# roahmlab/koopman-realizations

Measured on AMD Instinct MI355X. Metric: EDMD snapshot-pairs/sec (bilinear fit, 3-link arm, poly-3), higher is better.
Workload: dtype f64

## Files before the change

### koopman-realizations_amd/_ffi.py

```python
from __future__ import annotations

import ctypes as C
import os

import numpy as np

_HERE = os.path.dirname(os.path.abspath(__file__))
LIB_PATH = os.environ.get("KP_LIB_PATH") or os.path.join(_HERE, "libkoopman_hip.so")

KP_OK, KP_ERR_ARG, KP_ERR_HIP, KP_ERR_NOT_SPD, KP_ERR_QP_FAIL, KP_ERR_NOT_CONVERGED = 0, -1, -2, -3, -4, -5
MODEL = {"linear": 0, "bilinear": 1, "nonlinear": 2}
BLOCK = {"poly": 0, "fourier": 1, "gaussian": 2, "hermite": 3, "fourier_sparser": 4}
LIFT_FULL, LIFT_ECON, LIFT_ROW = 0, 1, 2

c_dp = C.POINTER(C.c_double)
c_ip = C.POINTER(C.c_int)
vp = C.c_void_p


class KpBasisDesc(C.Structure):
    _fields_ = [("model_type", C.c_int32), ("nzeta", C.c_int32), ("m", C.c_int32), ("n_blocks", C.c_int32),
                ("block_type", C.POINTER(C.c_int32)), ("block_count", C.POINTER(C.c_int32)),
                ("poly_exps", C.POINTER(C.c_uint8)), ("gauss_centres", c_dp),
                ("k_pcs", C.c_int32), ("pcs", c_dp)]
# ... 104 lines not shown
    "kp_nmpc_destroy": (C.c_int, [vp]),
}
TIMER_NMPC_SIM = 21

OBSERVER_SIGNATURES = {
    "kp_load_observe": (C.c_int, [vp, vp, C.c_int, c_dp, c_dp, C.c_int, C.c_int64, c_dp, c_dp, C.c_int,
                                  C.POINTER(C.c_int64), C.c_int64, C.POINTER(C.c_int32), C.POINTER(C.c_int64), C.c_int, c_dp,
                                  C.c_int, c_dp, c_dp, c_ip]),
}
OBS_RATE, OBS_PIN_LAST = 1, 2

CT_SIGNATURES = {
    "kp_logm": (C.c_int, [vp, C.c_int, C.c_int, c_dp, C.c_double, C.c_double, c_dp, c_ip, c_ip]),
    "kp_rollout_ct": (C.c_int, [vp, C.c_int, C.c_int, c_dp, c_dp, C.c_int, C.c_int, c_dp, c_dp, C.c_int, C.c_int, C.c_double,
                                C.c_double, C.c_double, c_dp, c_ip, c_ip, c_ip]),
    "kp_rollout_nl_ct": (C.c_int, [vp, vp, C.c_int, c_dp, c_dp, c_dp, C.c_int, C.c_double, C.c_double, C.c_double, c_dp, c_ip, c_ip,
                                   c_ip]),
}

class KpArmParams(C.Structure):
    _fields_ = [("Nmods", C.c_int), ("nlinks", C.c_int), ("l", C.c_double), ("k", C.c_double), ("d", C.c_double),
                ("m", C.c_double), ("i", C.c_double), ("g", C.c_double), ("ku", C.c_double)]


ARM_SIGNATURES = {
    "kp_arm_simulate": (C.c_int, [vp, C.POINTER(KpArmParams), C.c_int, C.c_int, C.c_int, c_dp, C.c_double, c_dp, c_dp, c_dp,
                                  C.c_double, C.c_double, c_dp, c_ip, c_ip, c_ip]),
}
ARM_MODE = {"zoh": 0, "interp": 1, "floor": 2, "restart": 3}

class KpRsysDims(C.Structure):
    _fields_ = [("num_terms", C.c_int), ("degree_x", C.c_int), ("degree_u", C.c_int)]


RSYS_SIGNATURES = {
    "kp_rsys_simulate": (C.c_int, [vp, C.POINTER(KpRsysDims), C.c_int, C.c_int, C.c_int, C.c_int, c_dp, c_dp, c_ip, c_ip, c_dp,
                                   c_dp, c_dp, C.c_int, C.c_double, C.c_double, c_dp, c_ip, c_ip, c_ip, C.POINTER(vp)]),
}
RSYS_MODE = {"span": 0, "restart": 1}

VALIDATE_SIGNATURES = {
    "kp_validate": (C.c_int, [vp, vp, C.c_int, C.c_int, C.c_int, C.c_int, C.c_int, C.c_int, C.c_int, c_dp, c_dp, C.c_int,
                              C.POINTER(C.c_int64), c_dp, c_dp, c_dp, c_dp, c_dp, C.c_int, c_dp, c_ip, c_dp]),
    "kp_validate_ct": (C.c_int, [vp, vp, C.c_int, C.c_int, C.c_int, C.c_int, C.c_int, C.c_int, C.c_int, c_dp, c_dp, C.c_int,
                                 C.POINTER(C.c_int64), c_dp, c_dp, c_dp, c_dp, c_dp, C.c_int, C.c_double, C.c_double, C.c_double,
                                 c_dp, c_ip, c_dp, c_ip, c_ip]),
}
HORIZON_SIGNATURES = {
    "kp_validate_horizon": (C.c_int, [vp, vp, C.c_int, C.c_int, C.c_int, C.c_int, C.c_int, C.c_int, c_dp, c_dp, C.c_int,
                                      C.POINTER(C.c_int64), c_dp, c_dp, c_dp, C.c_int, C.c_int, c_dp, C.POINTER(C.c_int64), c_ip]),
}
TIMER_HORIZON = 24
TIMER_HORIZON_TILE = 25
HORIZON_CHUNK = 8
VALIDATE_CHUNK = 128
VALIDATE_CT_CHUNK = 32
VALIDATE_CT_STAGE = 8192

SIM_SIGNATURES = {
    "kp_mpc_simulate": (C.c_int, [vp, vp, C.c_int, C.c_int, c_dp, C.c_int, c_dp, c_dp, C.c_int, c_dp, c_dp, c_dp, c_ip, c_ip]),
}
TIMER_MPC_SIM = 19

SPECTRUM_SIGNATURES = {
    "kp_eig": (C.c_int, [vp, C.c_int, C.c_int, c_dp, C.c_int, c_dp, c_dp, c_dp, c_ip, c_ip]),
}
TIMER_EIG = 22
TIMER_EIG_REGIME = 23
EIG_MAXN = 512
EIG_WAVE_MAX = 32
EIG_LDS_MAXN_VEC, EIG_LDS_MAXN_VAL = 99, 140

_lib = None


def lib():
    global _lib
    if _lib is None:
        if not os.path.exists(LIB_PATH):
            raise OSError(f"{LIB_PATH} not found: build it with `python -c 'import __graft_entry__ as g; g.build()'` "
                          "(make -C koopman-realizations_amd/csrc)")
        l = C.CDLL(LIB_PATH)
        for name, (res, args) in (SIGNATURES | NMPC_SIGNATURES | OBSERVER_SIGNATURES | CT_SIGNATURES | ARM_SIGNATURES
                                   | RSYS_SIGNATURES | VALIDATE_SIGNATURES | HORIZON_SIGNATURES | SIM_SIGNATURES | SPECTRUM_SIGNATURES).items():
            fn = getattr(l, name)
            fn.restype, fn.argtypes = res, args
        _lib = l
    return _lib


class KoopmanHipError(RuntimeError):
    def __init__(self, code, msg):
        super().__init__(f"libkoopman_hip error {code}: {msg}")
        self.code = code


def check(rc, ctx=None):
    if rc != KP_OK:
        msg = lib().kp_last_error(ctx)
        raise KoopmanHipError(rc, msg.decode() if msg else "")


def fcol(a, dtype=np.float64):
    return np.asfortranarray(np.asarray(a, dtype=dtype))


# ... 3 lines not shown
```

### koopman-realizations_amd/csrc/kp_context.hip

```cpp
#include <algorithm>
#include <cmath>
#include <cstring>
#include <mutex>

#include "kp_internal.h"

static std::mutex g_err_mu;
static std::string g_err;

void kp_set_global_error(const std::string& s) {
  std::lock_guard<std::mutex> l(g_err_mu);
  g_err = s;
}

void* kp_ctx::workspace(int slot, size_t bytes) {
  if (ws_bytes[slot] >= bytes && ws[slot]) return ws[slot];
  if (ws[slot]) (void)hipFree(ws[slot]);
  ws[slot] = nullptr;
  ws_bytes[slot] = 0;
  size_t want = bytes + bytes / 4 + 256;
  if (hipMalloc(&ws[slot], want) != hipSuccess) return nullptr;
  ws_bytes[slot] = want;
  return ws[slot];
}
// ... 82 lines not shown
  if (hipGetDeviceCount(&n) != hipSuccess) {
    (void)hipGetLastError();
    n = 0;
  }
  *count = n;
  return KP_OK;
}

extern "C" const char* kp_last_error(const kp_ctx* c) {
  if (c) return c->err.c_str();
  std::lock_guard<std::mutex> l(g_err_mu);
  static thread_local std::string copy;
  copy = g_err;
  return copy.c_str();
}

extern "C" int kp_device_info(const kp_ctx* c, char* name, int name_len, int* num_cu, int64_t* hbm) {
  if (!c) return KP_ERR_ARG;
  if (name && name_len > 0) {
    std::strncpy(name, c->name.c_str(), (size_t)name_len - 1);
    name[name_len - 1] = 0;
  }
  if (num_cu) *num_cu = c->num_cu;
  if (hbm) *hbm = c->hbm_bytes;
  return KP_OK;
}

void* kp_pinned_scratch(kp_ctx* ctx, size_t bytes) {
  if (ctx->pin_scratch_bytes >= bytes) return ctx->pin_scratch;
  if (ctx->pin_scratch) {
    (void)hipStreamSynchronize(ctx->stream);
    (void)hipHostFree(ctx->pin_scratch);
  }
  ctx->pin_scratch = nullptr;
  ctx->pin_scratch_bytes = 0;
  const size_t cap = (bytes + 4095) & ~(size_t)4095;
  if (hipHostMalloc(&ctx->pin_scratch, cap, hipHostMallocDefault) != hipSuccess) {
    ctx->pin_scratch = nullptr;
    return nullptr;
  }
  ctx->pin_scratch_bytes = cap;
  return ctx->pin_scratch;
}

int kp_dev_alloc_copy(kp_ctx* ctx, double** dst, const double* src, size_t n) {
  *dst = nullptr;
  if (!n) return KP_OK;
  KP_HIP(ctx, hipMalloc((void**)dst, n * 8));
  if (src) KP_HIP(ctx, hipMemcpy(*dst, src, n * 8, hipMemcpyHostToDevice));
  return KP_OK;
}

extern "C" int kp_timer_get(const kp_ctx* c, int which, double* ms) {
  if (!c || !ms || which < 0 || which >= 26) return KP_ERR_ARG;
  *ms = c->timers[which];
  return KP_OK;
}

extern "C" void* kp_stream(const kp_ctx* c) { return c ? (void*)c->stream : nullptr; }


static int upload(kp_ctx* ctx, void** dst, const void* src, size_t bytes) {
  *dst = nullptr;
  if (bytes == 0) return KP_OK;
  KP_HIP(ctx, hipMalloc(dst, bytes));
  KP_HIP(ctx, hipMemcpy(*dst, src, bytes, hipMemcpyHostToDevice));
  return KP_OK;
}

extern "C" int kp_basis_desc_dims(const kp_basis_desc* d, int* nvars_out, int* nfull_out, int* N_out, int* W_out) {
  if (!d || d->nzeta < 1 || d->m < 0 || d->model_type < 0 || d->model_type > 2 || d->n_blocks < 0 ||
      (d->n_blocks && (!d->block_type || !d->block_count)))
    return KP_ERR_ARG;
  const int nvars = d->nzeta + (d->model_type == KP_MODEL_NONLINEAR ? d->m : 0);
  double nf = nvars + 1.0;
  for (int b = 0; b < d->n_blocks; ++b) {
    const int c = d->block_count[b];
    if (c < 0) return KP_ERR_ARG;
    switch (d->block_type[b]) {
      case KP_BLOCK_POLY: case KP_BLOCK_HERMITE: case KP_BLOCK_FOURIER_SPARSER: case KP_BLOCK_GAUSSIAN: nf += c; break;
      case KP_BLOCK_FOURIER: nf += std::pow((double)(2 * c + 1), (double)nvars) - 1.0; break;
      default: return KP_ERR_ARG;
    }
    if (nf > 1e6) return KP_ERR_ARG;
  }
  const int nfull = (int)std::llround(nf);
  const int N = d->k_pcs > 0 ? d->k_pcs + nvars + 1 : nfull;
  if (nvars_out) *nvars_out = nvars;
  if (nfull_out) *nfull_out = nfull;
  if (N_out) *N_out = N;
  if (W_out) *W_out = d->model_type == KP_MODEL_BILINEAR ? N * (d->m + 1) : d->model_type == KP_MODEL_LINEAR ? N + d->m : N;
  return KP_OK;
}

extern "C" int kp_basis_create(kp_ctx* ctx, const kp_basis_desc* d, kp_basis** out) {
  if (!ctx || !d || !out) return KP_ERR_ARG;
  *out = nullptr;
  KP_HIP(ctx, hipSetDevice(ctx->device));
  if (d->model_type < 0 || d->model_type > 2) return ctx->fail(KP_ERR_ARG, "kp_basis_create: model_type");
  if (d->nzeta < 1 || d->m < 0) return ctx->fail(KP_ERR_ARG, "kp_basis_create: nzeta/m");
  int nvars = d->nzeta + (d->model_type == KP_MODEL_NONLINEAR ? d->m : 0);
  if (nvars > KP_MAX_VARS) return ctx->fail(KP_ERR_ARG, "kp_basis_create: too many variables (max 32)");
  std::vector<ColDesc> cols;
  for (int i = 0; i < nvars; ++i) cols.push_back({COL_VAR, i, 0, 0});
  int n_mono = 0, n_gauss = 0, max_deg = 1, fourier_deg = 0;
  for (int b = 0; b < d->n_blocks; ++b) {
    int cnt = d->block_count[b];
// ... 410 lines not shown
```

### koopman-realizations_amd/csrc/kp_gram3.hip

```cpp
#include <algorithm>
#include <cstdlib>
#include <type_traits>
#include <vector>

#include "kp_internal.h"

#ifndef KP_RAW_STEP
#define KP_RAW_STEP 1
#endif
#define KT3 8
#define NF3 3
#define RS3 240
#define YOFF3 96
#define ZOFF3 192
#define WOFF3 196
#define SOFF3 208
#define NIDMAX3 144
#define PST3 10
#define POWBUF3 (PST3 * NIDMAX3)
#define PSIBUF3 (KT3 * RS3)
#define PSI03 (2 * POWBUF3)
#define LDS3_DOUBLES (PSI03 + 2 * PSIBUF3)
#define PCS03 LDS3_DOUBLES
#define PCSMAX3 32
#define LDS3_PCS_DOUBLES (2 * YOFF3 * 16)
#define GC03 LDS3_DOUBLES
#define GAUSSMAX3 32
#ifndef KP_PCS_REGS
#define KP_PCS_REGS 24
#endif
#define GNZMAX3 8
#define LDS3_GAUSS_DOUBLES (GAUSSMAX3 * GNZMAX3)

#include "kp_gram3_args.h"
#include "kp_gram3_cover.h"
#include "kp_gram3_lift.h"

__device__ double kp_gram3_ones[KT3] = {1.0, 1.0, 1.0, 1.0, 1.0, 1.0, 1.0, 1.0};

template <int NQ, int BM, bool PCS, bool EXT = false, bool PRE = false, bool TUP = false, bool P3 = false, bool LO = false>
__global__ __launch_bounds__(256, 2) void kp_gram3_kernel(Gram3Args a) {
  constexpr int NWT = (BM + 1) * (BM + 2) / 2;
  static_assert(!P3 || (!PCS && !EXT && !PRE), "three-entry table: the in-kernel-lift monomial form");
  static_assert(!LO || (!PCS && !EXT && !PRE), "ordered lift slots: the in-kernel-lift monomial form");
  static_assert(!TUP || NWT % 2 == 0, "paired weights: an even number of weights (m = 3: 10 = 5 tuples, m = 2: 6 = 3 tuples)");
  auto wslot = [](int w) { return TUP ? 6 * (w & 1) + (w >> 1) : w - 1; };
  extern __shared__ __align__(16) double sm[];
  const BasisDev& b = a.b;
  const int tid = threadIdx.x;
  const int lane = tid & 63;
  const int wave = tid >> 6;
  const int per_xcd = gridDim.x / 8;
  const int logical = (int)blockIdx.x < per_xcd * 8 ? ((int)blockIdx.x % 8) * per_xcd + (int)blockIdx.x / 8 : (int)blockIdx.x;
  const int super = logical % a.nsuper;
  const int split = logical / a.nsuper;
  constexpr bool GRP = !PCS && !EXT && !PRE;
  const int fit = GRP ? __builtin_amdgcn_readfirstlane(split / a.nsplit_fit) : 0;
  const int split_local = split - fit * a.nsplit_fit;
  const double* const src_alpha = GRP ? a.grp[fit].alpha : a.alpha;
  const double* const src_beta = GRP ? a.grp[fit].beta : a.beta;
  const double* const src_u = GRP ? a.grp[fit].u : a.u;
  const int job = super * 4 + wave;
  const int nzm = b.nzeta + b.m;
  const int nrawrows = 2 * nzm;
  const int D = a.D;
  constexpr bool INL = !EXT && !PRE;
  const int RB = !INL ? D * PST3 : ((nrawrows + 1) * 62 + 4 * PST3 <= POWBUF3 ? 62 : 4 * PST3);
  const int CA = nrawrows * RB;

  const uint32_t* jd = a.desc + (size_t)job * (1 + NQ);
  const uint32_t jh = jd[0];
  const int lrow = (lane >> 4) * RS3, blk = (lane >> 2) & 3, lc = lane & 3;
  const int ao0 = PSI03 + lrow + 4 * (int)(jh & 255u) + lc;
  const int ao1 = PSI03 + lrow + 4 * (int)((jh >> 8) & 255u) + lc;
  const int qs = __builtin_amdgcn_readfirstlane((int)((jh >> 16) & 255u));
  int bo[NQ];
  int bo2[TUP ? NQ : 1];
#pragma unroll
  for (int q = 0; q < NQ; ++q) {
    const int g = (int)((jd[1 + q] >> (8 * (TUP ? (blk & 1) : blk))) & 255u);
    bo[q] = PSI03 + lrow + (g < a.G4 ? 4 * g : g < 2 * a.G4 ? YOFF3 + 4 * (g - a.G4) : ZOFF3) + lc;
    if (TUP) {
      const int g2 = (int)((jd[1 + q] >> (8 * (2 + (blk & 1)))) & 255u);
      bo2[q] = PSI03 + lrow + (g2 < a.G4 ? 4 * g2 : g2 < 2 * a.G4 ? YOFF3 + 4 * (g2 - a.G4) : ZOFF3) + lc;
    }
  }
  const int wo = PSI03 + lrow + WOFF3 + (TUP ? 6 * (blk >> 1) : 0);

  double acc[NQ][NWT];
#pragma unroll
  for (int q = 0; q < NQ; ++q)
#pragma unroll
    for (int w = 0; w < NWT; ++w) acc[q][w] = 0.0;

  auto item_setup = [&](int item, int (&fa_)[NF3], int& woff_) __attribute__((always_inline)) {
// ... 304 lines not shown
    const int nk = nf4 / 4;
#pragma unroll
    for (int kk = 0; kk < PREG; ++kk) {
      if (kk < nk) {
        const double av = sm[abase + 4 * kk];
        const double b1 = sm[bb1 + kk * 64];
        p0 = __builtin_amdgcn_mfma_f64_4x4x4f64(av, pcs_r[kk], p0, 0, 0, 0);
        p1 = __builtin_amdgcn_mfma_f64_4x4x4f64(av, b1, p1, 0, 0, 0);
      }
    }
#pragma unroll 3
    for (int kk = PREG; kk < nk; ++kk) {
      const double av = sm[abase + 4 * kk];
      const double b0 = sm[bbase + kk * 64], b1 = sm[bb1 + kk * 64];
      p0 = __builtin_amdgcn_mfma_f64_4x4x4f64(av, b0, p0, 0, 0, 0);
      p1 = __builtin_amdgcn_mfma_f64_4x4x4f64(av, b1, p1, 0, 0, 0);
    }
    const int crow = BUF * PSIBUF3 + PSI03 + (tid & (KT3 - 1)) * RS3 + ((tid / KT3) & 1) * YOFF3;
    const double one = sm[crow + b.nfull - 1];
    __syncthreads();
    {
      const int srow = BUF * PSIBUF3 + PSI03 + (4 * rg + (lane >> 4)) * RS3 + side * YOFF3;
      const int pc = 4 * blk + lc;
      if (pc < b.k_pcs) sm[srow + b.nzeta + pc] = p0;
      if (pc + 16 < b.k_pcs) sm[srow + b.nzeta + pc + 16] = p1;
    }
    if (tid < 2 * KT3) {
      sm[crow + b.N - 1] = one;
      for (int c = b.N; c < 4 * a.G4; ++c) sm[crow + c] = 0.0;
    }
    __syncthreads();
  };

  __syncthreads();
  if constexpr (PRE) {
    store_pre(B0{}, load_pre());
    __syncthreads();
  } else {
    if constexpr (INL) store_tb_v(B0{}, tb_v0, 0);
    else store_raw(B0{}, load_raw());
    lds_store_barrier();
#pragma unroll
    for (int i = 0; i < NCH; ++i) {
      lift_read(i, B0{});
      lift_write(i, B0{});
    }
    if constexpr (INL) store_tb_v(B1{}, tb_v1, 1);
    else store_raw(B1{}, load_raw());
    lds_store_barrier();
    if (PCS) project(B0{});
  }

  constexpr int NSTEP = (KT3 / 4) * NQ;
  constexpr int SP = NSTEP / NCH > 0 ? NSTEP / NCH : 1;
  constexpr int LAG = SP / 2 > 0 ? SP / 2 : 1;
  constexpr int PF_AHEAD = LO ? 2 : 3;
  constexpr int PF = NSTEP < PF_AHEAD ? NSTEP : PF_AHEAD;

  auto tile = [&](auto cur_c, auto qs_c) __attribute__((always_inline)) {
    constexpr int CUR = decltype(cur_c)::value;
    constexpr int QS = decltype(qs_c)::value;
    using NXT = std::integral_constant<int, 1 - CUR>;
    constexpr int PB = CUR * PSIBUF3;
    RawRegs rawreg;
    PreRegs prereg;
    if constexpr (LO) {
#pragma unroll
      for (int j = 0; j < NLS; ++j) {
#pragma unroll
        for (int f = 0; f < NF3; ++f)
          if (f < lift_nf(j)) asm volatile("" : "+v"(fsb[j][f]));
        asm volatile("" : "+v"(wsb[j]));
      }
    }
    constexpr int NAW = TUP ? NWT / 2 : NWT;
    double bvs[NSTEP];
    double bvs2[TUP ? NSTEP : 1];
    double aw[NAW];
    double wt[NAW];
    double av1 = 0.0;
    double avn0, avn1 = 0.0;
    auto weigh = [&](double av) __attribute__((always_inline)) {
#pragma unroll
      for (int w = 0; w < NAW; ++w) {
        aw[w] = (!TUP && w == 0) ? av : av * wt[w];
      }
    };
#pragma unroll
    for (int i = 0; i < PF; ++i) {
      bvs[i] = sm[PB + (i / NQ) * 4 * RS3 + bo[i % NQ]];
      if constexpr (TUP) bvs2[i] = sm[PB + (i / NQ) * 4 * RS3 + bo2[i % NQ]];
    }
    avn0 = sm[PB + ao0];
    if (QS < NQ) avn1 = sm[PB + ao1];
    auto load_wt = [&](int kk) __attribute__((always_inline)) {
      if constexpr (TUP) {
#pragma unroll
        for (int w = 0; w + 1 < NAW; w += 2) {
          const double2 v = *reinterpret_cast<const double2*>(&sm[PB + kk * 4 * RS3 + wo + w]);
          wt[w] = v.x;
          wt[w + 1] = v.y;
        }
        wt[NAW - 1] = sm[PB + kk * 4 * RS3 + wo + NAW - 1];
      } else {
#pragma unroll
        for (int w = 0; w < NWT - 1; w += 2) {
          const double2 v = *reinterpret_cast<const double2*>(&sm[PB + kk * 4 * RS3 + wo + w]);
          wt[w + 1] = v.x;
          if (w + 2 < NWT) wt[w + 2] = v.y;
        }
      }
    };
    load_wt(0);
#pragma unroll
    for (int step = 0; step < NSTEP; ++step) {
      const int kk = step / NQ, q = step % NQ;
      if (step == (NSTEP > KP_RAW_STEP ? KP_RAW_STEP : 0)) {
        if constexpr (PRE) prereg = load_pre();
        else if constexpr (INL) {
          store_tb(cur_c);
          load_tb();
        } else rawreg = load_raw();
      }
      if (q == 0) {
        weigh(avn0);
        if (QS < NQ) av1 = avn1;
        if (kk + 1 < KT3 / 4) {
          avn0 = sm[PB + (kk + 1) * 4 * RS3 + ao0];
          if (QS < NQ) avn1 = sm[PB + (kk + 1) * 4 * RS3 + ao1];
        }
      }
      if (QS < NQ && q == QS) weigh(av1);
      if (QS < NQ && QS > 1 && q == QS - 1) load_wt(kk);
      if (q == NQ - 1 && kk + 1 < KT3 / 4) load_wt(kk + 1);
      if (step + PF < NSTEP) {
        bvs[step + PF] = sm[PB + ((step + PF) / NQ) * 4 * RS3 + bo[(step + PF) % NQ]];
        if constexpr (TUP) bvs2[step + PF] = sm[PB + ((step + PF) / NQ) * 4 * RS3 + bo2[(step + PF) % NQ]];
      }
      const double bv = bvs[step];
      const double bv2 = TUP ? bvs2[step] : 0.0;
      if constexpr (TUP) {
#pragma unroll
        for (int w = 0; w < NAW; ++w) {
          acc[q][2 * w] = __builtin_amdgcn_mfma_f64_4x4x4f64(aw[w], bv, acc[q][2 * w], 0, 0, 0);
          acc[q][2 * w + 1] = __builtin_amdgcn_mfma_f64_4x4x4f64(aw[w], bv2, acc[q][2 * w + 1], 0, 0, 0);
        }
      } else {
#pragma unroll
        for (int w = 0; w < NWT; ++w) acc[q][w] = __builtin_amdgcn_mfma_f64_4x4x4f64(aw[w], bv, acc[q][w], 0, 0, 0);
      }
      if constexpr (!PRE) {
        if (step >= LAG && (step - LAG) % SP == 0 && (step - LAG) / SP < NCH) lift_write((step - LAG) / SP, NXT{});
        if (step % SP == 0 && step / SP < NCH) lift_read(step / SP, NXT{});
      }
      __builtin_amdgcn_sched_barrier(0);
    }
    if constexpr (!PRE) {
#pragma unroll
      for (int i = 0; i < NCH; ++i) {
        if (i * SP >= NSTEP) lift_read(i, NXT{});
        if (i * SP + LAG >= NSTEP) lift_write(i, NXT{});
      }
    }
    if constexpr (PRE) {
      store_pre(NXT{}, prereg);
      __syncthreads();
    } else {
      if constexpr (!INL) store_raw(cur_c, rawreg);
      lds_store_barrier();
    }
    if (PCS) project(NXT{});
  };
  auto run_tiles = [&](auto qs_c) __attribute__((always_inline)) {
    int t = 0;
    for (; t + 1 < nkt; t += 2) {
      tile(B0{}, qs_c);
      tile(B1{}, qs_c);
    }
    if (t < nkt) tile(B0{}, qs_c);
  };
  switch (qs) {
    case 1: run_tiles(std::integral_constant<int, 1>{}); break;
    case 2: run_tiles(std::integral_constant<int, (NQ >= 2 ? 2 : NQ)>{}); break;
    case 3: run_tiles(std::integral_constant<int, (NQ >= 3 ? 3 : NQ)>{}); break;
    case 4: run_tiles(std::integral_constant<int, (NQ >= 4 ? 4 : NQ)>{}); break;
    case 5: run_tiles(std::integral_constant<int, (NQ >= 5 ? 5 : NQ)>{}); break;
    default: run_tiles(std::integral_constant<int, NQ>{}); break;
  }

  double* dst = a.part + (((size_t)split * a.njobs + job) * NQ) * NWT * 64 + lane;
#pragma unroll
  for (int q = 0; q < NQ; ++q)
#pragma unroll
    for (int w = 0; w < NWT; ++w) dst[(q * NWT + w) * 64] = acc[q][w];
}

__global__ __launch_bounds__(1024) void kp_gram3_reduce_kernel(const double* __restrict__ part, int nsplit, int njobs, int NQ, int NWT,
                                                              int BM, const uint32_t* __restrict__ desc, int G4, int N, int W,
                                                              double* __restrict__ G, double* __restrict__ C, int tup,
                                                              const uint32_t* __restrict__ dst_off, const uint32_t* __restrict__ dst) {
  const int idx = blockIdx.x;
  int w = idx % NWT;
  const int jq = idx / NWT, q = jq % NQ, job = jq / NQ;
  const int l = threadIdx.x & 63, wv = threadIdx.x >> 6, nwv = blockDim.x >> 6;
  __shared__ double red[16][64];
  const size_t per_split = (size_t)njobs * NQ * NWT * 64;
  const double* src = part + (size_t)blockIdx.y * nsplit * per_split + (size_t)idx * 64 + l;
  G += (size_t)blockIdx.y * 2 * W * W;
  C += (size_t)blockIdx.y * 2 * W * W;
  double s0 = 0.0, s1 = 0.0, s2 = 0.0, s3 = 0.0;
  int p = wv;
  for (; p + 3 * nwv < nsplit; p += 4 * nwv) {
    const double v0 = src[(size_t)p * per_split], v1 = src[(size_t)(p + nwv) * per_split];
    const double v2 = src[(size_t)(p + 2 * nwv) * per_split], v3 = src[(size_t)(p + 3 * nwv) * per_split];
    s0 += v0; s1 += v1; s2 += v2; s3 += v3;
  }
  for (; p < nsplit; p += nwv) s0 += src[(size_t)p * per_split];
  red[wv][l] = (s0 + s1) + (s2 + s3);
  __syncthreads();
  if (wv) return;
  double s = red[0][l];
  for (int v = 1; v < nwv; ++v) s += red[v][l];
  const uint32_t* jd = desc + (size_t)job * (1 + NQ);
  const int ga = q < (int)((jd[0] >> 16) & 255u) ? (int)(jd[0] & 255u) : (int)((jd[0] >> 8) & 255u);
  int gsel = (l >> 2) & 3;
  if (tup) {
// ... 43 lines not shown
  int two_group_jobs = 0;
  uint32_t* desc = nullptr;
  uint32_t* dst_off = nullptr;
  uint32_t* dst = nullptr;
  kp_gram3_plan* cover = nullptr;
  bool cover_tried = false;
  uint32_t* lift = nullptr;
  bool lift_tried = false;
};

void kp_gram3_plan_free(kp_gram3_plan* p) {
  if (!p) return;
  kp_gram3_plan_free(p->cover);
  if (p->desc) (void)hipFree(p->desc);
  if (p->dst_off) (void)hipFree(p->dst_off);
  if (p->dst) (void)hipFree(p->dst);
  if (p->lift) (void)hipFree(p->lift);
  delete p;
}

static hipError_t plan3_upload(uint32_t** dev, const std::vector<uint32_t>& host) {
  hipError_t e = hipMalloc((void**)dev, std::max<size_t>(host.size(), 1) * 4);
  if (e == hipSuccess && !host.empty()) e = hipMemcpy(*dev, host.data(), host.size() * 4, hipMemcpyHostToDevice);
  return e;
}

static int make_plan3(kp_ctx* ctx, int N, int nwt, int nq_cap, kp_gram3_plan** out, int wpw = 4, int nq_force = 0) {
  kp_gram3_plan* p = new kp_gram3_plan();
  p->wpw = wpw;
  const int G4 = (N + 3) / 4;
  p->G4 = G4;
  size_t maxq = 0;
  const std::vector<std::vector<int>> rows = gram3_circulant_rows(G4, &maxq);
  Gram3JobsHost jobs;
  gram3_pack_rows(rows, G4, nwt, nq_cap, maxq, wpw, nq_force, &jobs);
  p->nq = jobs.nq;
  p->njobs = jobs.njobs;
  p->nsuper = jobs.njobs / wpw;
  p->two_group_jobs = gram3_two_group_jobs(jobs);
  hipError_t e = plan3_upload(&p->desc, jobs.desc);
  if (e != hipSuccess) {
    kp_gram3_plan_free(p);
    return ctx->fail(KP_ERR_HIP, std::string("kp_fit_gram: plan upload: ") + hipGetErrorString(e));
  }
  *out = p;
  return KP_OK;
}

static bool gram3_tup(int bm) {
  static const bool off = getenv("KP_GRAM3_NOTUP") != nullptr;
  return bm >= 2 && !off;
}

template <int NQ, int BM, bool PCS, bool EXT = false, bool PRE = false, bool TUP = false, bool P3 = false, bool LO = false>
static hipError_t launch3c(const Gram3Args& a, int grid, size_t lds, hipStream_t st) {
  static KpLdsCache lds_cache;
  {
    const size_t lds_max = (size_t)(LDS3_DOUBLES + (PCS ? LDS3_PCS_DOUBLES : 0) + (EXT ? LDS3_GAUSS_DOUBLES : 0)) * sizeof(double);
    hipError_t e = kp_ensure_lds(lds_cache, (const void*)kp_gram3_kernel<NQ, BM, PCS, EXT, PRE, TUP, P3, LO>, lds_max);
    if (e != hipSuccess) return e;
  }
  hipLaunchKernelGGL((kp_gram3_kernel<NQ, BM, PCS, EXT, PRE, TUP, P3, LO>), dim3(grid), dim3(256), lds, st, a);
  return hipGetLastError();
}

template <int NQ, int BM, bool PCS, bool EXT = false, bool PRE = false>
static hipError_t launch3b(const Gram3Args& a, int grid, size_t lds, hipStream_t st) {
  if constexpr (!PCS && !EXT && !PRE) {
    if (a.lift) return a.pow3 ? launch3c<NQ, BM, false, false, false, (BM >= 2), true, true>(a, grid, lds, st)
                              : launch3c<NQ, BM, false, false, false, (BM >= 2), false, true>(a, grid, lds, st);
    if (a.pow3) return launch3c<NQ, BM, false, false, false, (BM >= 2), true>(a, grid, lds, st);
  }
  if constexpr (BM >= 2) {
    if (gram3_tup(BM)) return launch3c<NQ, BM, PCS, EXT, PRE, true>(a, grid, lds, st);
  }
  return launch3c<NQ, BM, PCS, EXT, PRE, false>(a, grid, lds, st);
}

template <int NQ>
static hipError_t launch3(const Gram3Args& a, int bm, int grid, size_t lds, hipStream_t st) {
  if (a.pre) {
    switch (bm) {
      case 1: return launch3b<NQ, 1, false, false, true>(a, grid, lds, st);
      case 2: return launch3b<NQ, 2, false, false, true>(a, grid, lds, st);
      default: return launch3b<NQ, 3, false, false, true>(a, grid, lds, st);
    }
  }
  if (a.pcs) {
    if constexpr (NQ <= 4) {
      switch (bm) {
        case 1: return launch3b<NQ, 1, true>(a, grid, lds, st);
        case 2: return launch3b<NQ, 2, true>(a, grid, lds, st);
        default: return launch3b<NQ, 3, true>(a, grid, lds, st);
      }
    } else {
      return hipErrorInvalidValue;
    }
  }
  if (a.df > 0 || a.ng > 0) {
    switch (bm) {
      case 1: return launch3b<NQ, 1, false, true>(a, grid, lds, st);
      case 2: return launch3b<NQ, 2, false, true>(a, grid, lds, st);
      default: return launch3b<NQ, 3, false, true>(a, grid, lds, st);
    }
  }
  switch (bm) {
    case 1: return launch3b<NQ, 1, false>(a, grid, lds, st);
    case 2: return launch3b<NQ, 2, false>(a, grid, lds, st);
    default: return launch3b<NQ, 3, false>(a, grid, lds, st);
  }
}

static bool gram3_ext(const kp_basis* basis) {
  const BasisDev& b = basis->dev;
  return basis->fast_ext && (basis->ext_df > 0 || basis->ext_ng > 0) && b.k_pcs == 0 && basis->ext_ng <= GAUSSMAX3 &&
         (basis->ext_ng == 0 || b.nzeta <= GNZMAX3) && !getenv("KP_NO_GRAM3_EXT");
// ... 38 lines not shown

static int gram3_cover_mode() {
  static const int v = [] { const char* e = getenv("KP_GRAM3_COVER"); return e ? std::min(2, std::max(0, atoi(e))) : 1; }();
  return v;
}

static bool gram3_onea_on() {
  static const bool on = [] { const char* e = getenv("KP_GRAM3_ONEA"); return !e || atoi(e) != 0; }();
  return on;
}

static int gram3_cover_plan(kp_ctx* ctx, kp_basis* basis, kp_gram3_plan** out) {
  kp_gram3_plan& circ = *basis->plan3;
  *out = nullptr;
  if (!circ.cover_tried) {
    circ.cover_tried = true;
    const BasisDev& b = basis->dev;
    const int N = b.N, NWT = (b.m + 1) * (b.m + 2) / 2;
    if (circ.wpw != 4 || b.k_pcs != 0 || gram3_ext(basis) || !basis->fast || b.nfull != N || (int)basis->h_recipes.size() != N) return KP_OK;
    Gram3CoverHost cov;
    if (!gram3_cover_build(basis->h_recipes.data(), N, basis->pow_depth, NWT, 6, circ.wpw, &cov) || cov.jobs.njobs >= circ.njobs) return KP_OK;
    if (gram3_onea_on()) {
      Gram3CoverHost one;
      if (gram3_onea_build(basis->h_recipes.data(), N, basis->pow_depth, cov, &one) && one.jobs.nq == cov.jobs.nq && one.jobs.njobs <= cov.jobs.njobs) cov = std::move(one);
    }
    kp_gram3_plan* p = new kp_gram3_plan();
    p->G4 = circ.G4;
    p->two_group_jobs = gram3_two_group_jobs(cov.jobs);
    p->nq = cov.jobs.nq;
    p->njobs = cov.jobs.njobs;
    p->nsuper = cov.jobs.njobs / circ.wpw;
    p->cover_tried = true;
    hipError_t e = plan3_upload(&p->desc, cov.jobs.desc);
    if (e == hipSuccess) e = plan3_upload(&p->dst_off, cov.dst_off);
    if (e == hipSuccess) e = plan3_upload(&p->dst, cov.dst);
    if (e != hipSuccess) {
      kp_gram3_plan_free(p);
      circ.cover_tried = false;
      return ctx->fail(KP_ERR_HIP, std::string("kp_fit_gram: plan upload: ") + hipGetErrorString(e));
    }
    circ.cover = p;
  }
  *out = circ.cover;
  return KP_OK;
}

static bool gram3_pow3_on() {
  static const bool on = [] { const char* e = getenv("KP_GRAM3_POW3"); return !e || atoi(e) != 0; }();
  return on;
}

static bool gram3_lift_order_on() {
  static const bool on = [] { const char* e = getenv("KP_GRAM3_LIFT_ORDER"); return !e || atoi(e) != 0; }();
  return on;
}

static int gram3_lift_table(kp_ctx* ctx, kp_basis* basis, const uint32_t** out) {
  kp_gram3_plan& circ = *basis->plan3;
  *out = nullptr;
  if (!circ.lift_tried) {
    const BasisDev& b = basis->dev;
    Gram3LiftOrderHost lo;
    if (basis->fast && (int)basis->h_recipes.size() == b.nfull && gram3_lift_order_build(basis->h_recipes.data(), b.nfull, b.m, &lo)) {
      hipError_t e = plan3_upload(&circ.lift, lo.slot);
      if (e != hipSuccess) {
        if (circ.lift) (void)hipFree(circ.lift);
        circ.lift = nullptr;
        return ctx->fail(KP_ERR_HIP, std::string("kp_fit_gram: lift table upload: ") + hipGetErrorString(e));
      }
    }
    circ.lift_tried = true;
  }
  *out = circ.lift;
  return KP_OK;
}

static int gram3_plan_for(kp_ctx* ctx, kp_basis* basis, bool deferred, kp_gram3_plan** out) {
  int rc = gram3_plan(ctx, basis);
  if (rc) return rc;
  *out = basis->plan3;
  if (gram3_cover_mode() == 2 || (gram3_cover_mode() == 1 && deferred)) {
    kp_gram3_plan* cov = nullptr;
    rc = gram3_cover_plan(ctx, basis, &cov);
    if (rc) return rc;
    if (cov) *out = cov;
  }
  return KP_OK;
}

static int64_t gram3_slots(const kp_ctx* ctx, const kp_gram3_plan& plan, int* ncu_out = nullptr, int* wgpcu_out = nullptr) {
  int ncu = ctx->num_cu > 0 ? ctx->num_cu : 256;
  int wg_per_cu = plan.wpw == 8 ? 1 : 2;
  if (const char* ov = getenv("KP_GRAM3_WGPCU")) wg_per_cu = std::max(1, atoi(ov));
  if (ncu_out) *ncu_out = ncu;
  if (wgpcu_out) *wgpcu_out = wg_per_cu;
  return (int64_t)std::max(8, ncu) * wg_per_cu;
}

bool kp_gram3_groupable(kp_ctx* ctx, const kp_basis* basis_c, const kp_snapshots* s) {
  kp_basis* basis = const_cast<kp_basis*>(basis_c);
  const BasisDev& b = basis->dev;
  if (!(kp_gram3_applicable(basis) && b.k_pcs == 0 && !gram3_ext(basis) && !gram6_on() && s->nzeta == b.nzeta && s->m == b.m)) return false;
  kp_gram3_plan* plan = nullptr;
  if (gram3_plan_for(ctx, basis, true, &plan) != KP_OK || plan->wpw == 8) return false;
  static const int64_t max_kps = [] { const char* e = getenv("KP_GRAM_GROUP_MAX_KPS"); return e ? (int64_t)atoll(e) : (int64_t)512; }();
  const int64_t ktiles = (s->Ns + KT3 - 1) / KT3, nsplit = std::max<int64_t>(1, gram3_slots(ctx, *plan) / plan->nsuper);
// ... 39 lines not shown
  if (!part) return ctx->fail(KP_ERR_HIP, "kp_fit_gram: out of device memory");

  static const int64_t pre_min_ns = [] { const char* e = getenv("KP_GRAM3_PRELIFT_MIN_NS"); return e ? (int64_t)atoll(e) : (int64_t)6000; }();
  bool pre = gram3_prelift(basis) && s->Ns >= pre_min_ns;
  if (n > 1 && (pre || b.k_pcs > 0 || ext || plan.wpw == 8)) return ctx->fail(KP_ERR_ARG, "kp_fit_gram: these fits cannot share a launch");
  const int pre_rl = 8 * plan.G4 + 12;
  double* pre_buf = nullptr;
  if (pre) {
    const size_t pre_bytes = (size_t)ktiles * KT3 * pre_rl * 8;
    if (ctx->hbm_bytes > 0 && pre_bytes > (size_t)ctx->hbm_bytes / 4) pre = false;
    if (pre) {
      pre_buf = (double*)ctx->workspace(14, pre_bytes);
      if (!pre_buf) {
        (void)hipGetLastError();
        pre = false;
      }
    }
  }
  if (pre && !ext && !basis->d_pcsT) {
    if (hipMalloc(&basis->d_pcsT, (size_t)b.nfull * 32 * 8) != hipSuccess) return ctx->fail(KP_ERR_HIP, "kp_fit_gram: out of device memory");
    KP_HIP(ctx, kp_gram3_pcs_transpose_launch(b.pcs, b.nfull, b.k_pcs, (double*)basis->d_pcsT, ctx->stream));
  }
  const size_t lds = (size_t)(LDS3_DOUBLES + (b.k_pcs > 0 && !pre ? 2 * nfull4 * 16 : 0) + (ext && !pre ? LDS3_GAUSS_DOUBLES : 0)) * sizeof(double);

  Gram3Args a;
  a.b = b;
  a.alpha = s->alpha;
  a.beta = s->beta;
  a.u = s->u;
  a.Ns = s->Ns;
  a.G4 = plan.G4;
  a.nsuper = plan.nsuper;
  a.ktiles_per_split = kps;
  a.D = ext ? basis->ext_Dp + 2 * basis->ext_df : basis->pow_depth;
  a.recipes = (const uint32_t*)(ext ? basis->d_recipes_ext : basis->d_recipes);
  a.Dp = ext ? basis->ext_Dp : basis->pow_depth;
  a.df = ext ? basis->ext_df : 0;
  a.ng = ext ? basis->ext_ng : 0;
  a.centres = b.centres;
  a.desc = plan.desc;
  a.part = part;
  a.njobs = plan.njobs;
  a.pcs = b.k_pcs > 0 && !pre ? b.pcs : nullptr;
  a.nfull4 = nfull4;
  a.pre = pre_buf;
  a.pre_rl = pre_rl;
  a.nsplit_fit = nsplit;
  for (int f = 0; f < n; ++f) a.grp[f] = Gram3Src{ss[f]->alpha, ss[f]->beta, ss[f]->u};
  a.pow3 = !pre && b.k_pcs == 0 && !ext && plan.wpw == 4 && basis->pow_depth <= 3 && (BM < 2 || gram3_tup(BM)) && gram3_pow3_on();
  if (!pre && b.k_pcs == 0 && !ext && plan.wpw == 4 && (BM < 2 || gram3_tup(BM)) && gram3_lift_order_on()) {
    int rc = gram3_lift_table(ctx, basis, &a.lift);
    if (rc) return rc;
  }
  const int grid = plan.nsuper * nsplit * n;
  if (!ctx->ring_timing) KP_HIP(ctx, hipEventRecord(ctx->ev0, ctx->stream));
  hipEvent_t ev_start = ctx->evp[0], ev_end = ctx->evp[1];
  const bool timed = !ctx->ring_timing || (ctx->ring_group && n > 1) || (ctx->ring_skip++ & 3) == 0;
  hipEvent_t ev_red = nullptr;
  if (ctx->ring_timing && timed) {
    ev_start = ctx->ring[2 * ctx->ring_pos];
    ev_end = ctx->ring[2 * ctx->ring_pos + 1];
    ctx->ring_members[ctx->ring_pos] = n;
    ctx->ring_has_red[ctx->ring_pos] = false;
    if (ctx->ring_group && n > 1) {
      ev_red = ctx->ring_red[ctx->ring_pos];
      ctx->ring_has_red[ctx->ring_pos] = ev_red != nullptr;
    }
    ctx->ring_pos = (ctx->ring_pos + 1) % 64;
    if (ctx->ring_n < 64) ++ctx->ring_n;
  }
  if (timed) KP_HIP(ctx, hipEventRecord(ev_start, ctx->stream));
  hipError_t e;
  if (pre && ext)
    KP_HIP(ctx, kp_gram3_prelift_ext_launch(BM, s->alpha, s->beta, s->u, s->Ns, ktiles * KT3, b.nzeta, basis->ext_Dp, basis->ext_df, basis->ext_ng, b.nfull, plan.G4,
                                            (const uint32_t*)basis->d_recipes_ext, b.centres, pre_buf, pre_rl, ctx->stream));
  else if (pre)
    KP_HIP(ctx, kp_gram3_prelift_launch(BM, s->alpha, s->beta, s->u, s->Ns, ktiles * KT3, b.nzeta, basis->pow_depth, b.nfull, b.k_pcs, N, plan.G4,
                                        (const uint32_t*)basis->d_recipes, (const double*)basis->d_pcsT, pre_buf, pre_rl, ctx->stream));
  if (plan.wpw == 8) e = kp_gram6_launch_kernel(a, plan.nq, grid, ctx->stream);
  else switch (plan.nq) {
    case 1: e = launch3<1>(a, BM, grid, lds, ctx->stream); break;
    case 2: e = launch3<2>(a, BM, grid, lds, ctx->stream); break;
    case 3: e = launch3<3>(a, BM, grid, lds, ctx->stream); break;
    case 4: e = launch3<4>(a, BM, grid, lds, ctx->stream); break;
    case 5: e = launch3<5>(a, BM, grid, lds, ctx->stream); break;
    default: e = launch3<6>(a, BM, grid, lds, ctx->stream); break;
  }
  KP_HIP(ctx, e);
  if (timed) KP_HIP(ctx, hipEventRecord(ev_end, ctx->stream));
  hipLaunchKernelGGL(kp_gram3_reduce_kernel, dim3(plan.njobs * plan.nq * NWT, n), dim3(nsplit >= 128 ? 1024 : nsplit >= 32 ? 512 : 256), 0, ctx->stream, part, nsplit, plan.njobs,
                     plan.nq, NWT, BM, plan.desc, plan.G4, N, W, GC_dev, GC_dev + (size_t)W * W, plan.wpw != 8 && gram3_tup(BM) ? 1 : 0, plan.dst_off, plan.dst);
  KP_HIP(ctx, hipGetLastError());
  if (ev_red) KP_HIP(ctx, hipEventRecord(ev_red, ctx->stream));
  if (!ctx->ring_timing) {
    KP_HIP(ctx, hipEventRecord(ctx->ev1, ctx->stream));
    KP_HIP(ctx, hipEventRecord(ctx->evp[2], ctx->stream));
  }
  ctx->gram_flops_per_pair = (double)W * (W + 1) + 2.0 * W * W;
  ctx->timers[10] = (double)plan.njobs * plan.nq * NWT * 128.0 + (b.k_pcs > 0 && !pre ? (double)plan.nsuper * nfull4 * 128.0 : 0.0);
  ctx->timers[16] = (pre || ext || plan.wpw == 8) ? 0.0 : a.pow3 ? 3.0 : 4.0;
  ctx->timers[20] = a.lift ? 1.0 : 0.0;
  ctx->timers[15] = (double)plan.two_group_jobs;
  return KP_OK;
}

int kp_gram3_launch(kp_ctx* ctx, const kp_basis* basis, const kp_snapshots* s, double* GC_dev, bool cover) { return gram3_launch_n(ctx, basis, &s, 1, GC_dev, cover); }

int kp_gram3_launch_group(kp_ctx* ctx, const kp_basis* basis, const kp_snapshots* const* ss, int n, double* GC_dev) {
  return gram3_launch_n(ctx, basis, ss, n, GC_dev, true);
}


__global__ __launch_bounds__(256) void kp_gram3_linear_gather_kernel(const double* __restrict__ GCb, int N, int m, int Wb, double* __restrict__ GC) {
  const int W = N + m;
  const int e = blockIdx.x * 256 + threadIdx.x;
  if (e >= 2 * W * W) return;
  const int which = e / (W * W), r = e - which * W * W, i = r % W, j = r / W;
  const int bi = i < N ? i : (i - N + 1) * N + N - 1, bj = j < N ? j : (j - N + 1) * N + N - 1;
  GC[e] = GCb[(size_t)which * Wb * Wb + (size_t)bj * Wb + bi];
}

static kp_basis* gram3_shadow(const kp_basis* basis_c) {
  kp_basis* basis = const_cast<kp_basis*>(basis_c);
  if (!basis->shadow_bil) {
    kp_basis* sh = new kp_basis(*basis);
    sh->dev.model_type = KP_MODEL_BILINEAR;
    sh->dev.W = sh->dev.N * (sh->dev.m + 1);
    sh->plan = nullptr; sh->plan2 = nullptr; sh->plan3 = nullptr; sh->plan5 = nullptr; sh->shadow_bil = nullptr;
    sh->d_pcsT = nullptr;
    basis->shadow_bil = sh;
  }
  return basis->shadow_bil;
}

void kp_gram3_shadow_free(kp_basis* basis) {
  if (!basis) return;
  if (basis->shadow_bil) {
    kp_gram3_plan_free(basis->shadow_bil->plan3);
    if (basis->shadow_bil->d_pcsT) (void)hipFree(basis->shadow_bil->d_pcsT);
    delete basis->shadow_bil;
    basis->shadow_bil = nullptr;
  }
  if (basis->shadow_full) {
    kp_gram_plan_free(basis->shadow_full->plan);
    kp_gram2_plan_free(basis->shadow_full->plan2);
    kp_gram5_plan_free(basis->shadow_full->plan5);
    delete basis->shadow_full;
    basis->shadow_full = nullptr;
  }
}

bool kp_gram3_linear_applicable(const kp_basis* basis) {
  const BasisDev& b = basis->dev;
  if (b.model_type != KP_MODEL_LINEAR || b.k_pcs <= 0 || b.m < 1 || getenv("KP_NO_GRAM3_LINEAR")) return false;
// ... 107 lines not shown
```

### koopman-realizations_amd/csrc/kp_gram3_args.h

```cpp
#pragma once
#include "kp_internal.h"

struct Gram3Src { const double *alpha, *beta, *u; };

struct Gram3Args {
  BasisDev b;
  const double* alpha;
  const double* beta;
  const double* u;
  int64_t Ns;
  int G4;
  int nsuper;
  int ktiles_per_split;
  int D;
  const uint32_t* recipes;
  const uint32_t* desc;
  double* part;
  int njobs;
  const double* pcs;
  int nfull4;
  int Dp, df, ng;
  const double* centres;
  const double* pre = nullptr;
  int pre_rl = 0;
  int nsplit_fit = 1 << 30;
  Gram3Src grp[KP_GRAM_GROUP_MAX] = {};
  bool pow3 = false;
  const uint32_t* lift = nullptr;
};

bool kp_gram6_serves(int nq, int G4);
hipError_t kp_gram6_launch_kernel(const Gram3Args& a, int nq, int grid, hipStream_t st);

hipError_t kp_gram3_pcs_transpose_launch(const double* pcs, int nfull, int k, double* pcsT, hipStream_t st);
hipError_t kp_gram3_prelift_launch(int BM, const double* alpha, const double* beta, const double* u, int64_t Ns, int64_t Ns_pad, int nzeta, int D, int nfull, int k_pcs,
                                   int N, int G4, const uint32_t* recipes, const double* pcsT, double* out, int rl, hipStream_t st);
hipError_t kp_gram3_prelift_ext_launch(int BM, const double* alpha, const double* beta, const double* u, int64_t Ns, int64_t Ns_pad, int nzeta, int Dp, int df, int ng,
                                       int nfull, int G4, const uint32_t* recipes, const double* centres, double* out, int rl, hipStream_t st);
```

### koopman-realizations_amd/csrc/kp_internal.h

```cpp
#pragma once
#include <hip/hip_runtime.h>
#include <stdint.h>
#include <atomic>
#include <mutex>
#include <string>
#include <utility>
#include <vector>

#include "koopman_hip.h"

#define KP_MAX_VARS 32
#define KP_GRAM_GROUP_MAX 8

void kp_set_global_error(const std::string& s);
void kp_traj_device_blocks(kp_traj* t, double** blocks);
struct kp_comm_state;

struct kp_stage;

struct kp_ctx {
  int device = 0;
  kp_stage* stage = nullptr;
  std::vector<void*> host_blocks;
  std::vector<std::pair<void*, size_t>> traj_pool;
  std::mutex host_mu;
  hipStream_t stream = nullptr;
  hipEvent_t ev0 = nullptr, ev1 = nullptr;
  hipEvent_t evp[6] = {nullptr};
  hipStream_t stream2 = nullptr;
  hipEvent_t ev_gram_done = nullptr;
  bool async_pending = false;
  int kring_cap = 128;
  int async_count = 0;
  bool batch_closed = true;
  bool kres_is_ring = false;
  const void* pend_basis = nullptr;
  int64_t pend_Ns = 0;
  int pend_W = 0;
  int pend_solves = 0, pend_first = 0;
  hipEvent_t ev_solve0 = nullptr, ev_solve1 = nullptr;
  int* sticky_info = nullptr;
  const kp_snapshots* pend_grams[KP_GRAM_GROUP_MAX] = {};
  int pend_ngrams = 0;
  const kp_basis* pend_gram_basis = nullptr;
  double* pend_gram_gc = nullptr;
  bool ring_timing = false;
  bool ring_group = false;
  unsigned ring_skip = 0;
  hipEvent_t ring[2 * 64] = {};
  int ring_pos = 0, ring_n = 0;
  hipEvent_t ring_red[64] = {};
  int ring_members[64] = {};
  bool ring_has_red[64] = {};
  kp_comm_state* comm = nullptr;
  std::atomic<bool> comm_abandoned{false};
  bool gc_preloaded = false;
  bool reduce_grams = false;
  bool test_hooks = false;
  void* pin_scratch = nullptr;
  size_t pin_scratch_bytes = 0;
  double* pin_small = nullptr;
  int num_cu = 0;
  int64_t hbm_bytes = 0;
  std::string name;
  mutable std::string err;
  double timers[26] = {0};
  double gram_flops_per_pair = 0;
  void* ws[21] = {nullptr};
  size_t ws_bytes[21] = {0};
  int last_rank = -1;
  double last_pivot_ratio = 1.0;
  double* Kres = nullptr;
  size_t Kres_bytes = 0;
  int Kres_W = 0, Kres_n = 0;
  double* GC = nullptr;
  size_t GC_bytes = 0;
  int GC_W = 0;

  int fail(int code, const std::string& s) const {
    err = s;
    kp_set_global_error(s);
    return code;
  }
  void* workspace(int slot, size_t bytes);
};

#define KP_HIP(ctx, expr)                                                                  \
  do {                                                                                     \
    hipError_t _e = (expr);                                                                \
    if (_e != hipSuccess)                                                                  \
      return (ctx)->fail(KP_ERR_HIP, std::string(#expr) + ": " + hipGetErrorString(_e));   \
  } while (0)

enum : int { COL_VAR = 0, COL_MONO = 1, COL_FOURIER = 2, COL_GAUSS = 3, COL_CONST = 4, COL_HERMITE = 5, COL_FSPARSE = 6 };

struct ColDesc {
  int32_t kind;
  int32_t arg;
  int32_t aux;
  int32_t pad;
};

struct BasisDev {
  int model_type, nzeta, m, nvars;
  int nfull, N, W, k_pcs;
  const ColDesc* cols;
  const uint8_t* exps;
  const double* centres;
  const double* pcs;
};

struct KpLdsCache { size_t set[32] = {}; };
inline hipError_t kp_ensure_lds(KpLdsCache& c, const void* func, size_t lds) {
  int dev = -1;
  if (hipGetDevice(&dev) != hipSuccess || dev < 0 || dev >= 32) return hipFuncSetAttribute(func, hipFuncAttributeMaxDynamicSharedMemorySize, (int)lds);
  if (lds > c.set[dev]) {
    hipError_t e = hipFuncSetAttribute(func, hipFuncAttributeMaxDynamicSharedMemorySize, (int)lds);
    if (e != hipSuccess) return e;
    c.set[dev] = lds;
// ... 210 lines not shown
```

Measured before the change: 336.9 million.

## Move gram3 tile barrier earlier and prefetch next tile's LDS operands

New measurement: 345.0 million (median of 6 runs). 1.02x the previous value.

```diff
diff --git a/koopman-realizations_amd/_ffi.py b/koopman-realizations_amd/_ffi.py
--- a/koopman-realizations_amd/_ffi.py
+++ b/koopman-realizations_amd/_ffi.py
@@ -180,6 +180,7 @@
 }
 TIMER_HORIZON = 24
 TIMER_HORIZON_TILE = 25
+TIMER_GRAM3_EARLY_BARRIER = 26
 HORIZON_CHUNK = 8
 VALIDATE_CHUNK = 128
 VALIDATE_CT_CHUNK = 32
diff --git a/koopman-realizations_amd/csrc/kp_context.hip b/koopman-realizations_amd/csrc/kp_context.hip
--- a/koopman-realizations_amd/csrc/kp_context.hip
+++ b/koopman-realizations_amd/csrc/kp_context.hip
@@ -158,7 +158,7 @@
 }
 
 extern "C" int kp_timer_get(const kp_ctx* c, int which, double* ms) {
-  if (!c || !ms || which < 0 || which >= 26) return KP_ERR_ARG;
+  if (!c || !ms || which < 0 || which >= 27) return KP_ERR_ARG;
   *ms = c->timers[which];
   return KP_OK;
 }
diff --git a/koopman-realizations_amd/csrc/kp_gram3.hip b/koopman-realizations_amd/csrc/kp_gram3.hip
--- a/koopman-realizations_amd/csrc/kp_gram3.hip
+++ b/koopman-realizations_amd/csrc/kp_gram3.hip
@@ -38,9 +38,35 @@
 
 __device__ double kp_gram3_ones[KT3] = {1.0, 1.0, 1.0, 1.0, 1.0, 1.0, 1.0, 1.0};
 
-template <int NQ, int BM, bool PCS, bool EXT = false, bool PRE = false, bool TUP = false, bool P3 = false, bool LO = false>
+#ifndef KP_GRAM3_EB_BEHIND
+#define KP_GRAM3_EB_BEHIND 0
+#endif
+struct Gram3TileTiming {
+  int pf;
+  int sp, lag;
+  int bs;
+};
+constexpr Gram3TileTiming gram3_tile_timing(int nq, bool lo, bool eb) {
+  const int nstep = (KT3 / 4) * nq, nch = 3;
+  const int pf_ahead = lo ? 2 : 3;
+  const int pf = nstep < pf_ahead ? nstep : pf_ahead;
+  const int sp = nstep / nch > 0 ? nstep / nch : 1;
+  const int lag = sp / 2 > 0 ? sp / 2 : 1;
+  if (eb && lo) {
+    const int behind = KP_GRAM3_EB_BEHIND > 0 && KP_GRAM3_EB_BEHIND < pf ? KP_GRAM3_EB_BEHIND : pf;
+    const int bs = nstep - 1 - behind;
+    for (int s = sp; s >= 2; --s) {
+      const int l = lag < s ? lag : s;
+      if (bs >= (KT3 / 4 - 1) * nq && (nch - 1) * s + l <= bs) return {pf, s, l, bs};
+    }
+  }
+  return {pf, sp, lag, -1};
+}
+
+template <int NQ, int BM, bool PCS, bool EXT = false, bool PRE = false, bool TUP = false, bool P3 = false, bool LO = false, bool EB = false>
 __global__ __launch_bounds__(256, 2) void kp_gram3_kernel(Gram3Args a) {
   constexpr int NWT = (BM + 1) * (BM + 2) / 2;
+  static_assert(!EB || (!PCS && !EXT && !PRE), "early tile barrier: the in-kernel-lift monomial form");
   static_assert(!P3 || (!PCS && !EXT && !PRE), "three-entry table: the in-kernel-lift monomial form");
   static_assert(!LO || (!PCS && !EXT && !PRE), "ordered lift slots: the in-kernel-lift monomial form");
   static_assert(!TUP || NWT % 2 == 0, "paired weights: an even number of weights (m = 3: 10 = 5 tuples, m = 2: 6 = 3 tuples)");
@@ -451,16 +477,55 @@
   }
 
   constexpr int NSTEP = (KT3 / 4) * NQ;
-  constexpr int SP = NSTEP / NCH > 0 ? NSTEP / NCH : 1;
-  constexpr int LAG = SP / 2 > 0 ? SP / 2 : 1;
-  constexpr int PF_AHEAD = LO ? 2 : 3;
-  constexpr int PF = NSTEP < PF_AHEAD ? NSTEP : PF_AHEAD;
+  constexpr Gram3TileTiming TT = gram3_tile_timing(NQ, LO, EB);
+  constexpr int SP = TT.sp;
+  constexpr int LAG = TT.lag;
+  constexpr int PF = TT.pf;
+  constexpr int BS = TT.bs;
+  constexpr bool EBT = BS >= 0;
+  static_assert(!EBT || (EB && BS < NSTEP - 1 && BS >= (KT3 / 4 - 1) * NQ && BS >= KP_RAW_STEP && (NCH - 1) * SP + LAG <= BS && LAG <= SP),
+                "early barrier: behind the table store, the last lift store and the last k-step's first step, in front of the tile's last step");
+  constexpr int NAW = TUP ? NWT / 2 : NWT;
+  double bvs[NSTEP];
+  double bvs2[TUP ? NSTEP : 1];
+  double wt[NAW];
+  double avn0 = 0.0, avn1 = 0.0;
+  auto load_b = [&](int pb, int i) __attribute__((always_inline)) {
+    bvs[i] = sm[pb + (i / NQ) * 4 * RS3 + bo[i % NQ]];
+    if constexpr (TUP) bvs2[i] = sm[pb + (i / NQ) * 4 * RS3 + bo2[i % NQ]];
+  };
+  auto load_wt = [&](int pb, int kk) __attribute__((always_inline)) {
+    if constexpr (TUP) {
+#pragma unroll
+      for (int w = 0; w + 1 < NAW; w += 2) {
+        const double2 v = *reinterpret_cast<const double2*>(&sm[pb + kk * 4 * RS3 + wo + w]);
+        wt[w] = v.x;
+        wt[w + 1] = v.y;
+      }
+      wt[NAW - 1] = sm[pb + kk * 4 * RS3 + wo + NAW - 1];
+    } else {
+#pragma unroll
+      for (int w = 0; w < NWT - 1; w += 2) {
+        const double2 v = *reinterpret_cast<const double2*>(&sm[pb + kk * 4 * RS3 + wo + w]);
+        wt[w + 1] = v.x;
+        if (w + 2 < NWT) wt[w + 2] = v.y;
+      }
+    }
+  };
+  auto head_reads = [&](int pb, bool two_groups) __attribute__((always_inline)) {
+#pragma unroll
+    for (int i = 0; i < PF; ++i) load_b(pb, i);
+    avn0 = sm[pb + ao0];
+    if (two_groups) avn1 = sm[pb + ao1];
+    load_wt(pb, 0);
+  };
 
   auto tile = [&](auto cur_c, auto qs_c) __attribute__((always_inline)) {
     constexpr int CUR = decltype(cur_c)::value;
     constexpr int QS = decltype(qs_c)::value;
     using NXT = std::integral_constant<int, 1 - CUR>;
     constexpr int PB = CUR * PSIBUF3;
+    constexpr int NPB = (1 - CUR) * PSIBUF3;
     RawRegs rawreg;
     PreRegs prereg;
     if constexpr (LO) {
@@ -472,45 +537,15 @@
         asm volatile("" : "+v"(wsb[j]));
       }
     }
-    constexpr int NAW = TUP ? NWT / 2 : NWT;
-    double bvs[NSTEP];
-    double bvs2[TUP ? NSTEP : 1];
     double aw[NAW];
-    double wt[NAW];
     double av1 = 0.0;
-    double avn0, avn1 = 0.0;
     auto weigh = [&](double av) __attribute__((always_inline)) {
 #pragma unroll
       for (int w = 0; w < NAW; ++w) {
         aw[w] = (!TUP && w == 0) ? av : av * wt[w];
       }
     };
-#pragma unroll
-    for (int i = 0; i < PF; ++i) {
-      bvs[i] = sm[PB + (i / NQ) * 4 * RS3 + bo[i % NQ]];
-      if constexpr (TUP) bvs2[i] = sm[PB + (i / NQ) * 4 * RS3 + bo2[i % NQ]];
-    }
-    avn0 = sm[PB + ao0];
-    if (QS < NQ) avn1 = sm[PB + ao1];
-    auto load_wt = [&](int kk) __attribute__((always_inline)) {
-      if constexpr (TUP) {
-#pragma unroll
-        for (int w = 0; w + 1 < NAW; w += 2) {
-          const double2 v = *reinterpret_cast<const double2*>(&sm[PB + kk * 4 * RS3 + wo + w]);
-          wt[w] = v.x;
-          wt[w + 1] = v.y;
-        }
-        wt[NAW - 1] = sm[PB + kk * 4 * RS3 + wo + NAW - 1];
-      } else {
-#pragma unroll
-        for (int w = 0; w < NWT - 1; w += 2) {
-          const double2 v = *reinterpret_cast<const double2*>(&sm[PB + kk * 4 * RS3 + wo + w]);
-          wt[w + 1] = v.x;
-          if (w + 2 < NWT) wt[w + 2] = v.y;
-        }
-      }
-    };
-    load_wt(0);
+    if constexpr (!EBT) head_reads(PB, QS < NQ);
 #pragma unroll
     for (int step = 0; step < NSTEP; ++step) {
       const int kk = step / NQ, q = step % NQ;
@@ -530,11 +565,19 @@
         }
       }
       if (QS < NQ && q == QS) weigh(av1);
-      if (QS < NQ && QS > 1 && q == QS - 1) load_wt(kk);
-      if (q == NQ - 1 && kk + 1 < KT3 / 4) load_wt(kk + 1);
-      if (step + PF < NSTEP) {
-        bvs[step + PF] = sm[PB + ((step + PF) / NQ) * 4 * RS3 + bo[(step + PF) % NQ]];
-        if constexpr (TUP) bvs2[step + PF] = sm[PB + ((step + PF) / NQ) * 4 * RS3 + bo2[(step + PF) % NQ]];
+      const int wstep = kk * NQ + QS - 1;
+      if (QS < NQ && QS > 1 && step == (EBT && wstep > BS ? BS : wstep)) load_wt(PB, kk);
+      if (q == NQ - 1) {
+        if (kk + 1 < KT3 / 4) load_wt(PB, kk + 1);
+        else if constexpr (EBT) {
+          load_wt(NPB, 0);
+          avn0 = sm[NPB + ao0];
+          if (QS < NQ) avn1 = sm[NPB + ao1];
+        }
+      }
+      if (step + PF < NSTEP) load_b(PB, step + PF);
+      else if constexpr (EBT) {
+        if (step > BS) load_b(NPB, step + PF - NSTEP);
       }
       const double bv = bvs[step];
       const double bv2 = TUP ? bvs2[step] : 0.0;
@@ -552,6 +595,13 @@
         if (step >= LAG && (step - LAG) % SP == 0 && (step - LAG) / SP < NCH) lift_write((step - LAG) / SP, NXT{});
         if (step % SP == 0 && step / SP < NCH) lift_read(step / SP, NXT{});
       }
+      if constexpr (EBT) {
+        if (step == BS) {
+          lds_store_barrier();
+#pragma unroll
+          for (int s = NSTEP - PF; s <= BS; ++s) load_b(NPB, s + PF - NSTEP);
+        }
+      }
       __builtin_amdgcn_sched_barrier(0);
     }
     if constexpr (!PRE) {
@@ -564,13 +614,14 @@
     if constexpr (PRE) {
       store_pre(NXT{}, prereg);
       __syncthreads();
-    } else {
+    } else if constexpr (!EBT) {
       if constexpr (!INL) store_raw(cur_c, rawreg);
       lds_store_barrier();
     }
     if (PCS) project(NXT{});
   };
   auto run_tiles = [&](auto qs_c) __attribute__((always_inline)) {
+    if constexpr (EBT) head_reads(0, decltype(qs_c)::value < NQ);
     int t = 0;
     for (; t + 1 < nkt; t += 2) {
       tile(B0{}, qs_c);
@@ -720,16 +771,24 @@
   return bm >= 2 && !off;
 }
 
-template <int NQ, int BM, bool PCS, bool EXT = false, bool PRE = false, bool TUP = false, bool P3 = false, bool LO = false>
-static hipError_t launch3c(const Gram3Args& a, int grid, size_t lds, hipStream_t st) {
+template <int NQ, int BM, bool PCS, bool EXT = false, bool PRE = false, bool TUP = false, bool P3 = false, bool LO = false, bool EB = false>
+static hipError_t launch3d(const Gram3Args& a, int grid, size_t lds, hipStream_t st) {
   static KpLdsCache lds_cache;
   {
     const size_t lds_max = (size_t)(LDS3_DOUBLES + (PCS ? LDS3_PCS_DOUBLES : 0) + (EXT ? LDS3_GAUSS_DOUBLES : 0)) * sizeof(double);
-    hipError_t e = kp_ensure_lds(lds_cache, (const void*)kp_gram3_kernel<NQ, BM, PCS, EXT, PRE, TUP, P3, LO>, lds_max);
+    hipError_t e = kp_ensure_lds(lds_cache, (const void*)kp_gram3_kernel<NQ, BM, PCS, EXT, PRE, TUP, P3, LO, EB>, lds_max);
     if (e != hipSuccess) return e;
   }
-  hipLaunchKernelGGL((kp_gram3_kernel<NQ, BM, PCS, EXT, PRE, TUP, P3, LO>), dim3(grid), dim3(256), lds, st, a);
+  hipLaunchKernelGGL((kp_gram3_kernel<NQ, BM, PCS, EXT, PRE, TUP, P3, LO, EB>), dim3(grid), dim3(256), lds, st, a);
   return hipGetLastError();
+}
+
+template <int NQ, int BM, bool PCS, bool EXT = false, bool PRE = false, bool TUP = false, bool P3 = false, bool LO = false>
+static hipError_t launch3c(const Gram3Args& a, int grid, size_t lds, hipStream_t st) {
+  if constexpr (!PCS && !EXT && !PRE && gram3_tile_timing(NQ, LO, true).bs >= 0) {
+    if (a.eb) return launch3d<NQ, BM, PCS, EXT, PRE, TUP, P3, LO, true>(a, grid, lds, st);
+  }
+  return launch3d<NQ, BM, PCS, EXT, PRE, TUP, P3, LO, false>(a, grid, lds, st);
 }
 
 template <int NQ, int BM, bool PCS, bool EXT = false, bool PRE = false>
@@ -874,6 +933,11 @@
 
 static bool gram3_lift_order_on() {
   static const bool on = [] { const char* e = getenv("KP_GRAM3_LIFT_ORDER"); return !e || atoi(e) != 0; }();
+  return on;
+}
+
+static bool gram3_early_barrier_on() {
+  static const bool on = [] { const char* e = getenv("KP_GRAM3_EARLY_BARRIER"); return !e || atoi(e) != 0; }();
   return on;
 }
 
@@ -1019,6 +1083,8 @@
     int rc = gram3_lift_table(ctx, basis, &a.lift);
     if (rc) return rc;
   }
+  a.eb = !pre && b.k_pcs == 0 && !ext && plan.wpw == 4 && gram3_early_barrier_on() && gram3_tile_timing(plan.nq, a.lift != nullptr, true).bs >= 0 &&
+         (plan.two_group_jobs == 0 || plan.nq < 6 || BM < 3);
   const int grid = plan.nsuper * nsplit * n;
   if (!ctx->ring_timing) KP_HIP(ctx, hipEventRecord(ctx->ev0, ctx->stream));
   hipEvent_t ev_start = ctx->evp[0], ev_end = ctx->evp[1];
@@ -1067,6 +1133,7 @@
   ctx->timers[10] = (double)plan.njobs * plan.nq * NWT * 128.0 + (b.k_pcs > 0 && !pre ? (double)plan.nsuper * nfull4 * 128.0 : 0.0);
   ctx->timers[16] = (pre || ext || plan.wpw == 8) ? 0.0 : a.pow3 ? 3.0 : 4.0;
   ctx->timers[20] = a.lift ? 1.0 : 0.0;
+  ctx->timers[26] = a.eb ? 1.0 : 0.0;
   ctx->timers[15] = (double)plan.two_group_jobs;
   return KP_OK;
 }
diff --git a/koopman-realizations_amd/csrc/kp_gram3_args.h b/koopman-realizations_amd/csrc/kp_gram3_args.h
--- a/koopman-realizations_amd/csrc/kp_gram3_args.h
+++ b/koopman-realizations_amd/csrc/kp_gram3_args.h
@@ -27,6 +27,7 @@
   Gram3Src grp[KP_GRAM_GROUP_MAX] = {};
   bool pow3 = false;
   const uint32_t* lift = nullptr;
+  bool eb = false;
 };
 
 bool kp_gram6_serves(int nq, int G4);
diff --git a/koopman-realizations_amd/csrc/kp_internal.h b/koopman-realizations_amd/csrc/kp_internal.h
--- a/koopman-realizations_amd/csrc/kp_internal.h
+++ b/koopman-realizations_amd/csrc/kp_internal.h
@@ -64,7 +64,7 @@
   int64_t hbm_bytes = 0;
   std::string name;
   mutable std::string err;
-  double timers[26] = {0};
+  double timers[27] = {0};
   double gram_flops_per_pair = 0;
   void* ws[21] = {nullptr};
   size_t ws_bytes[21] = {0};
```
